# opencb/hpg-variant

Hardware: AMD Instinct MI355X
Metric: variants/s chi2 assoc (higher is better)
Workload: dtype u8

## Files before the change

hpg-variant_amd/csrc/hpgv_kernels.h:

```cpp
#pragma once
#include <hip/hip_runtime.h>
#include <stdint.h>

namespace hpgv {

__device__ __forceinline__ uint32_t nib_nonzero(uint32_t x) {
    uint32_t y = x | (x << 1);
    y = y | (y << 2);
    return y & 0x88888888u;
}
__device__ __forceinline__ uint32_t nib_not_f(uint32_t x) { return nib_nonzero(~x); }

__device__ __forceinline__ int wave_sum(int v) {
    v += __builtin_amdgcn_update_dpp(0, v, 0xB1, 0xF, 0xF, true);
    v += __builtin_amdgcn_update_dpp(0, v, 0x4E, 0xF, 0xF, true);
    v += __builtin_amdgcn_update_dpp(0, v, 0x141, 0xF, 0xF, true);
    v += __builtin_amdgcn_update_dpp(0, v, 0x140, 0xF, 0xF, true);
    return __builtin_amdgcn_readlane(v, 0) + __builtin_amdgcn_readlane(v, 16) +
           __builtin_amdgcn_readlane(v, 32) + __builtin_amdgcn_readlane(v, 48);
}

template <bool NT>
__device__ __forceinline__ uint4 load16(const uint4 *p);
template <bool NT>
__device__ __forceinline__ uint4 load16o(const uint8_t *__restrict__ base, uint32_t byte_off) {
    return load16<NT>(reinterpret_cast<const uint4 *>(base + byte_off));
}
template <bool NT>
__device__ __forceinline__ uint4 load16(const uint4 *p) {
    if constexpr (NT) {
        typedef uint32_t u32x4 __attribute__((ext_vector_type(4)));
        u32x4 t = __builtin_nontemporal_load(reinterpret_cast<const u32x4 *>(p));
        return make_uint4(t.x, t.y, t.z, t.w);
    } else {
        return *p;
    }
}

template <bool NT, int U, bool X>
__device__ __forceinline__ void assoc_row(const uint8_t *__restrict__ row, int lane, int chunksA,
                                          int chunks, uint32_t &pnz, uint32_t &pnnf, uint32_t &pbnz) {
    for (int base = 0; base < chunks; base += 64 * U) {
        uint4 q[U];
#pragma unroll
        for (int u = 0; u < U; ++u) {
            const int c = base + u * 64 + lane;
            q[u] = make_uint4(~0u, ~0u, ~0u, ~0u);
            if (c < chunks) q[u] = load16o<NT>(row, (uint32_t)c * 16u);
        }
#pragma unroll
        for (int u = 0; u < U; ++u) {
            const int c = base + u * 64 + lane;
            const uint32_t sh = (c < chunksA) ? 0u : 16u;
            const uint32_t w[4] = {q[u].x, q[u].y, q[u].z, q[u].w};
            uint32_t nz = 0, nnf = 0, bnz = 0;
#pragma unroll
            for (int k = 0; k < 4; ++k) {
                const uint32_t ind = nib_nonzero(w[k]);
                nz += __builtin_popcount(ind);
                nnf += __builtin_popcount(nib_not_f(w[k]));
                if constexpr (X) bnz += __builtin_popcount(ind & (ind >> 4) & 0x08080808u);
            }
            pnz += nz << sh;
            pnnf += nnf << sh;
            if constexpr (X) pbnz += bnz << sh;
        }
    }
}

__device__ __forceinline__ void assoc_row_finish(bool x_row, int lane, int TA, int TU, uint32_t pnz,
                                                 uint32_t pnnf, uint32_t pbnz, int4 *__restrict__ dst) {
    const int nzA = wave_sum((int)(pnz & 0xFFFFu)), nzU = wave_sum((int)(pnz >> 16));
    const int nfA = wave_sum((int)(pnnf & 0xFFFFu)), nfU = wave_sum((int)(pnnf >> 16));
    int4 out;
    if (!x_row) {
        out.x = TA - nzA;
        out.y = nzA + nfA - TA;
        out.z = TU - nzU;
        out.w = nzU + nfU - TU;
    } else {
        const int bA = wave_sum((int)(pbnz & 0xFFFFu)), bU = wave_sum((int)(pbnz >> 16));
        const int validA = nfA >> 1, validU = nfU >> 1;
        const int xxA = bA - (TA / 2 - validA), xxU = bU - (TU / 2 - validU);
        out.x = (TA - nzA) - validA + xxA;
        out.y = xxA;
        out.z = (TU - nzU) - validU + xxU;
        out.w = xxU;
    }
    if (lane == 0) *dst = out;
}

template <bool NT, int U, bool STRIDED>
__global__ __launch_bounds__(256) void k_assoc_scan(const uint8_t *__restrict__ gt, size_t pitch,
                                                    int n_variants, int chunksA, int chunks,
                                                    const uint8_t *__restrict__ is_x,
                                                    int4 *__restrict__ counts, int vpw) {
    const int lane = threadIdx.x & 63;
    const long wave = (long)blockIdx.x * (blockDim.x >> 6) + (threadIdx.x >> 6);
    const int slots = ((chunks + 64 * U - 1) / (64 * U)) * (64 * U);
    const int TA = 32 * chunksA;
    const int TU = 32 * (slots - chunksA);
    long v, v_end, v_step;
    if constexpr (STRIDED) { v = wave; v_end = n_variants; v_step = (long)gridDim.x * (blockDim.x >> 6); }
    else { v = wave * vpw; v_end = v + vpw < n_variants ? v + vpw : n_variants; v_step = 1; }

    for (; v < v_end; v += v_step) {
        const uint8_t *row = gt + (size_t)v * pitch;
        const bool x_row = (is_x != nullptr) && (__builtin_amdgcn_readfirstlane((int)is_x[v]) != 0);
        uint32_t pnz = 0, pnnf = 0, pbnz = 0;
        if (x_row) assoc_row<NT, U, true>(row, lane, chunksA, chunks, pnz, pnnf, pbnz);
        else       assoc_row<NT, U, false>(row, lane, chunksA, chunks, pnz, pnnf, pbnz);
        assoc_row_finish(x_row, lane, TA, TU, pnz, pnnf, pbnz, counts + v);
    }
}

struct AssocAcc { uint32_t pnz, pnnf, pbnz; };

template <int U, bool X>
__device__ __forceinline__ AssocAcc assoc_count_tile(const uint4 (&q)[U], int base, int lane, int chunksA,
                                                     AssocAcc a) {
#pragma unroll
    for (int u = 0; u < U; ++u) {
        const int c = base + u * 64 + lane;
        const uint32_t sh = (c < chunksA) ? 0u : 16u;
        const uint32_t w[4] = {q[u].x, q[u].y, q[u].z, q[u].w};
        uint32_t nz = 0, nnf = 0, bnz = 0;
#pragma unroll
        for (int k = 0; k < 4; ++k) {
            const uint32_t ind = nib_nonzero(w[k]);
            nz += __builtin_popcount(ind);
            nnf += __builtin_popcount(nib_not_f(w[k]));
            if constexpr (X) bnz += __builtin_popcount(ind & (ind >> 4) & 0x08080808u);
        }
        a.pnz += nz << sh;
        a.pnnf += nnf << sh;
        if constexpr (X) a.pbnz += bnz << sh;
    }
    return a;
}

template <bool NT, int U>
__device__ __forceinline__ void assoc_issue_tile(uint4 (&q)[U], const uint8_t *__restrict__ g0, size_t pitch,
                                                 int t, int ipr, int chunks, int lane) {
    const int r = t / ipr, base = (t - r * ipr) * 64 * U;
    const uint8_t *row = g0 + (size_t)r * pitch;
#pragma unroll
    for (int u = 0; u < U; ++u) {
        const int c = base + u * 64 + lane;
        q[u] = make_uint4(~0u, ~0u, ~0u, ~0u);
        if (c < chunks) q[u] = load16o<NT>(row, (uint32_t)c * 16u);
    }
}

template <int U>
__device__ __forceinline__ AssocAcc assoc_consume_tile(const uint4 (&q)[U], AssocAcc a, int t, int ipr, long v_begin,
                                                       int lane, int chunksA, int TA, int TU,
                                                       const uint8_t *__restrict__ is_x, int4 *__restrict__ counts) {
    const int r = t / ipr, it = t - r * ipr;
    const long v = v_begin + r;
    const bool x_row = (is_x != nullptr) && (__builtin_amdgcn_readfirstlane((int)is_x[v]) != 0);
    if (x_row) a = assoc_count_tile<U, true>(q, it * 64 * U, lane, chunksA, a);
    else       a = assoc_count_tile<U, false>(q, it * 64 * U, lane, chunksA, a);
    if (it == ipr - 1) {
        assoc_row_finish(x_row, lane, TA, TU, a.pnz, a.pnnf, a.pbnz, counts + v);
        a.pnz = a.pnnf = a.pbnz = 0;
    }
    return a;
}

template <bool NT, int U, int WAVES>
__global__ __launch_bounds__(256, WAVES) void k_assoc_scan_pipe(const uint8_t *__restrict__ gt, size_t pitch,
                                                         int n_variants, int chunksA, int chunks,
                                                         const uint8_t *__restrict__ is_x,
                                                         int4 *__restrict__ counts, int vpw) {
    const int lane = threadIdx.x & 63;
    const long wave = (long)blockIdx.x * (blockDim.x >> 6) + (threadIdx.x >> 6);
    const long v_begin = wave * vpw;
    if (v_begin >= n_variants) return;
    const int rows = (int)((v_begin + vpw <= n_variants) ? vpw : (n_variants - v_begin));
    const int ipr = (chunks + 64 * U - 1) / (64 * U);
    const int slots = ipr * 64 * U;
    const int TA = 32 * chunksA, TU = 32 * (slots - chunksA);
    const int n_tiles = rows * ipr;
    const uint8_t *g0 = gt + (size_t)v_begin * pitch;
    AssocAcc acc = {0u, 0u, 0u};
    uint4 qa[U], qb[U];
    assoc_issue_tile<NT, U>(qa, g0, pitch, 0, ipr, chunks, lane);
    for (int t = 0; t < n_tiles; t += 2) {
        if (t + 1 < n_tiles) assoc_issue_tile<NT, U>(qb, g0, pitch, t + 1, ipr, chunks, lane);
        acc = assoc_consume_tile<U>(qa, acc, t, ipr, v_begin, lane, chunksA, TA, TU, is_x, counts);
        if (t + 1 < n_tiles) {
            if (t + 2 < n_tiles) assoc_issue_tile<NT, U>(qa, g0, pitch, t + 2, ipr, chunks, lane);
            acc = assoc_consume_tile<U>(qb, acc, t + 1, ipr, v_begin, lane, chunksA, TA, TU, is_x, counts);
        }
    }
}

__device__ __forceinline__ double chisq_p_value(double x) {
    if (x != x) return x;
    if (x <= 0.0) return 1.0;
    const double y = x / 2.0;
    double P;
    if (y > 0.5) P = 1.0 - erfc(sqrt(y));
    else         P = erf(sqrt(y));
    return 1.0 - P;
}

__device__ __forceinline__ double assoc_odds(int A1, int A2, int U1, int U2) {
    return (A2 == 0 || U1 == 0) ? __builtin_nan("") : ((double)A1 / A2) * ((double)U2 / U1);
}

__device__ __forceinline__ double assoc_chisq_value(int a, int c, int b, int d) {
    const double total = a + c + b + d;
    const double t_aff = a + c, t_un = b + d, t_1 = a + b, t_2 = c + d;
    const double e_a1 = (t_aff * t_1) / total;
    const double e_a2 = (t_aff * t_2) / total;
    const double e_u1 = (t_un * t_1) / total;
    const double e_u2 = (t_un * t_2) / total;
    return ((a - e_a1) * (a - e_a1)) / e_a1 + ((c - e_a2) * (c - e_a2)) / e_a2 +
           ((b - e_u1) * (b - e_u1)) / e_u1 + ((d - e_u2) * (d - e_u2)) / e_u2;
}

static __global__ __launch_bounds__(256) void k_assoc_chisq(const int4 *__restrict__ counts, int n,
                                                     double *__restrict__ odds,
                                                     double *__restrict__ chisq,
                                                     double *__restrict__ pval) {
    const int i = blockIdx.x * blockDim.x + threadIdx.x;
    if (i >= n) return;
    const int4 c4 = counts[i];
    const int a = c4.x, c = c4.y, b = c4.z, d = c4.w;
    const double x = assoc_chisq_value(a, c, b, d);
    odds[i] = assoc_odds(a, c, b, d);
    chisq[i] = x;
    pval[i] = chisq_p_value(x);
}

__device__ __forceinline__ double wave_sum_f64(double v) {
#pragma unroll
    for (int off = 32; off > 0; off >>= 1) v += __shfl_xor(v, off);
    return v;
}
__device__ __forceinline__ double wave_max_f64(double v) {
#pragma unroll
    for (int off = 32; off > 0; off >>= 1) { const double o = __shfl_xor(v, off); v = o > v ? o : v; }
    return v;
}

__device__ const double k_exp2_j64[64] = {
    0x1.0000000000000p+0, 0x1.02c9a3e778061p+0, 0x1.059b0d3158574p+0, 0x1.0874518759bc8p+0,
    0x1.0b5586cf9890fp+0, 0x1.0e3ec32d3d1a2p+0, 0x1.11301d0125b51p+0, 0x1.1429aaea92de0p+0,
    0x1.172b83c7d517bp+0, 0x1.1a35beb6fcb75p+0, 0x1.1d4873168b9aap+0, 0x1.2063b88628cd6p+0,
    0x1.2387a6e756238p+0, 0x1.26b4565e27cddp+0, 0x1.29e9df51fdee1p+0, 0x1.2d285a6e4030bp+0,
    0x1.306fe0a31b715p+0, 0x1.33c08b26416ffp+0, 0x1.371a7373aa9cbp+0, 0x1.3a7db34e59ff7p+0,
    0x1.3dea64c123422p+0, 0x1.4160a21f72e2ap+0, 0x1.44e086061892dp+0, 0x1.486a2b5c13cd0p+0,
    0x1.4bfdad5362a27p+0, 0x1.4f9b2769d2ca7p+0, 0x1.5342b569d4f82p+0, 0x1.56f4736b527dap+0,
    0x1.5ab07dd485429p+0, 0x1.5e76f15ad2148p+0, 0x1.6247eb03a5585p+0, 0x1.6623882552225p+0,
    0x1.6a09e667f3bcdp+0, 0x1.6dfb23c651a2fp+0, 0x1.71f75e8ec5f74p+0, 0x1.75feb564267c9p+0,
    0x1.7a11473eb0187p+0, 0x1.7e2f336cf4e62p+0, 0x1.82589994cce13p+0, 0x1.868d99b4492edp+0,
    0x1.8ace5422aa0dbp+0, 0x1.8f1ae99157736p+0, 0x1.93737b0cdc5e5p+0, 0x1.97d829fde4e50p+0,
    0x1.9c49182a3f090p+0, 0x1.a0c667b5de565p+0, 0x1.a5503b23e255dp+0, 0x1.a9e6b5579fdbfp+0,
    0x1.ae89f995ad3adp+0, 0x1.b33a2b84f15fbp+0, 0x1.b7f76f2fb5e47p+0, 0x1.bcc1e904bc1d2p+0,
    0x1.c199bdd85529cp+0, 0x1.c67f12e57d14bp+0, 0x1.cb720dcef9069p+0, 0x1.d072d4a07897cp+0,
    0x1.d5818dcfba487p+0, 0x1.da9e603db3285p+0, 0x1.dfc97337b9b5fp+0, 0x1.e502ee78b3ff6p+0,
    0x1.ea4afa2a490dap+0, 0x1.efa1bee615a27p+0, 0x1.f50765b6e4540p+0, 0x1.fa7c1819e90d8p+0,
};
__device__ __forceinline__ double fisher_exp(double e, const double *tab ) {
    const double kf = __builtin_rint(e * 0x1.71547652b82fep+6);
    double r = __builtin_fma(-kf, 0x1.62e42fe000000p-7, e);
    r = __builtin_fma(-kf, 0x1.f473de6af278fp-36, r);
    const int ki = (int)kf;
    const double tj = tab[ki & 63];
    double q = __builtin_fma(r, 1.0 / 120.0, 1.0 / 24.0);
    q = __builtin_fma(r, q, 1.0 / 6.0);
    q = __builtin_fma(r, q, 0.5);
    q = __builtin_fma(r * r, q, r);
    const double y = __builtin_fma(tj, q, tj);
    return e < -1100.0 ? 0.0 : __builtin_ldexp(y, ki >> 6);
}

struct FisherTab {
    const double *lf; const double *xt ; double konst; int r1, c1, d0;
    __device__ __forceinline__ double at(uint32_t byte_off) const { return *reinterpret_cast<const double *>(reinterpret_cast<const char *>(lf) + byte_off); }
    __device__ __forceinline__ double e(int x) const {
        const uint32_t x8 = (uint32_t)x << 3;
        return konst - at(x8) - at(((uint32_t)r1 << 3) - x8) - at(((uint32_t)c1 << 3) - x8) - at(((uint32_t)d0 << 3) + x8);
    }
    __device__ __forceinline__ double p(int x) const { return fisher_exp(e(x), xt); }
    __device__ __forceinline__ void e2(int x, double *e0, double *e1) const {
        const char *b = reinterpret_cast<const char *>(lf) - 16;
        double2 q0, q1, q2, q3;
        __builtin_memcpy(&q0, b + ((uint32_t)(x + 2) << 3), 16);
        __builtin_memcpy(&q1, b + ((uint32_t)(r1 - x + 1) << 3), 16);
        __builtin_memcpy(&q2, b + ((uint32_t)(c1 - x + 1) << 3), 16);
        __builtin_memcpy(&q3, b + ((uint32_t)(d0 + x + 2) << 3), 16);
        *e0 = konst - q0.x - q1.y - q2.y - q3.x;
        *e1 = konst - q0.y - q1.x - q2.x - q3.y;
    }
};

template <int W> __device__ __forceinline__ int sub_lane(int lane) { return lane & (W - 1); }
template <int W> __device__ __forceinline__ uint64_t sub_ballot(bool pred, int lane) {
    const uint64_t b = __ballot(pred);
    if constexpr (W == 64) { (void)lane; return b; }
    else return (b >> (lane & ~(W - 1))) & ((1ull << W) - 1ull);
}
template <int W> __device__ __forceinline__ double sub_sum_f64(double v) {
#pragma unroll
    for (int off = W / 2; off > 0; off >>= 1) v += __shfl_xor(v, off);
    return v;
}
template <int W> __device__ __forceinline__ double sub_first_f64(double v, int lane) { return __shfl(v, lane & ~(W - 1)); }

template <int W>
__device__ __forceinline__ void fisher_boundaries(const FisherTab &T, double thr , int L1, int R1, int L2, int R2, int lane,
                                                  int *xL, int *xR) {
    const int sl = sub_lane<W>(lane);
    while (R1 - L1 > W || R2 - L2 > W) {
        const bool go1 = R1 - L1 > W, go2 = R2 - L2 > W;
        const int step1 = (R1 - L1 + W - 1) / W, step2 = (R2 - L2 + W - 1) / W;
        const int x1 = L1 + sl * step1, x2 = L2 + sl * step2;
        const double v1 = (go1 && x1 < R1) ? T.e(x1) : 0.0;
        const double v2 = (go2 && x2 < R2) ? T.e(x2) : 0.0;
        if (go1) {
            const int j = __builtin_popcountll(sub_ballot<W>(x1 < R1 && v1 <= thr, lane));
            const int xj = L1 + j * step1;
            const int nL = (j == 0) ? L1 : L1 + (j - 1) * step1 + 1, nR = (j == W || xj >= R1) ? R1 : xj;
            L1 = nL; R1 = nR;
        }
        if (go2) {
            const int j = __builtin_popcountll(sub_ballot<W>(x2 < R2 && v2 > thr, lane));
            const int xj = L2 + j * step2;
            const int nL = (j == 0) ? L2 : L2 + (j - 1) * step2 + 1, nR = (j == W || xj >= R2) ? R2 : xj;
            L2 = nL; R2 = nR;
        }
    }
    const int x1 = L1 + sl, x2 = L2 + sl;
    const double v1 = x1 < R1 ? T.e(x1) : 0.0, v2 = x2 < R2 ? T.e(x2) : 0.0;
    *xL = L1 + __builtin_popcountll(sub_ballot<W>(x1 < R1 && v1 <= thr, lane));
    *xR = L2 + __builtin_popcountll(sub_ballot<W>(x2 < R2 && v2 > thr, lane));
}

template <int W>
__device__ __forceinline__ double fisher_tails(const FisherTab &T, int xL, int xR, int lo, int hi, int lane, double rel_cut) {
    const int sl = sub_lane<W>(lane);
    double partL = 0.0, partR = 0.0, cutL = 0.0, cutR = 0.0;
    bool onL = true, onR = true;
    for (int k = 0; onL || onR; ++k) {
        const int firstL = xL - 1 - 2 * W * k, firstR = xR + 2 * W * k;
        if (firstL < lo) onL = false;
        if (firstR > hi) onR = false;
        const int a = firstL - 2 * sl, b = firstR + 2 * sl;
        double eL0 = -2000.0, eL1 = -2000.0, eR0 = -2000.0, eR1 = -2000.0;
        if (onL && a >= lo) { double lo_e, hi_e; T.e2(a - 1, &lo_e, &hi_e); eL0 = hi_e; if (a - 1 >= lo) eL1 = lo_e; }
        if (onR && b <= hi) { double lo_e, hi_e; T.e2(b, &lo_e, &hi_e); eR0 = lo_e; if (b + 1 <= hi) eR1 = hi_e; }
        const double sL0 = fisher_exp(eL0, T.xt), sL1 = fisher_exp(eL1, T.xt), sR0 = fisher_exp(eR0, T.xt), sR1 = fisher_exp(eR1, T.xt);
        partL += sL0 + sL1; partR += sR0 + sR1;
        if (k == 0) { cutL = rel_cut * sub_first_f64<W>(sL0, lane); cutR = rel_cut * sub_first_f64<W>(sR0, lane); }
        if (onL && sub_ballot<W>(sL0 > cutL || sL1 > cutL, lane) == 0ull) onL = false;
        if (onR && sub_ballot<W>(sR0 > cutR || sR1 > cutR, lane) == 0ull) onR = false;
    }
    return sub_sum_f64<W>(partL + partR);
}

template <int W>
__device__ __forceinline__ bool fisher_boundary_windows(const FisherTab &T, double thr , int mode, int obs, int lane,
                                                        int *L1, int *R1, int *L2, int *R2) {
    const int sl = sub_lane<W>(lane);
    const int g1 = obs <= mode ? obs + 1 : 2 * mode - obs + 1, g2 = obs <= mode ? 2 * mode - obs : obs;
    int w1 = g1 - W / 2, w2 = g2 - W / 2;
    w1 = w1 > *R1 - W ? *R1 - W : w1; w1 = w1 < *L1 ? *L1 : w1;
    w2 = w2 > *R2 - W ? *R2 - W : w2; w2 = w2 < *L2 ? *L2 : w2;
    const int x1 = w1 + sl, x2 = w2 + sl;
    const bool in1 = x1 < *R1, in2 = x2 < *R2;
    const double v1 = in1 ? T.e(x1) : 0.0, v2 = in2 ? T.e(x2) : 0.0;
    const int n1 = __builtin_popcountll(sub_ballot<W>(in1, lane)), n2 = __builtin_popcountll(sub_ballot<W>(in2, lane));
    const int c1 = __builtin_popcountll(sub_ballot<W>(in1 && v1 <= thr, lane)), c2 = __builtin_popcountll(sub_ballot<W>(in2 && v2 > thr, lane));
    bool ok = true;
    if (c1 == 0 && w1 > *L1) { *R1 = w1; ok = false; }
    else if (c1 == n1 && w1 + n1 < *R1) { *L1 = w1 + n1; ok = false; }
    else { *L1 = w1 + c1; *R1 = w1 + c1; }
    if (c2 == 0 && w2 > *L2) { *R2 = w2; ok = false; }
    else if (c2 == n2 && w2 + n2 < *R2) { *L2 = w2 + n2; ok = false; }
    else { *L2 = w2 + c2; *R2 = w2 + c2; }
    return ok;
}

template <int W>
__device__ __forceinline__ double fisher_sub(int a, int b, int c, int d, const double *__restrict__ lf,
                                             const double *exp_tab , double rel_cut, int lane) {
    const int sl = sub_lane<W>(lane);
    const int r1 = a + b, r2 = c + d, c1 = a + c, nn = r1 + r2;
    const int lo = (c1 - r2) > 0 ? (c1 - r2) : 0;
    const int hi = r1 < c1 ? r1 : c1;
    FisherTab T;
    T.lf = lf; T.xt = exp_tab; T.r1 = r1; T.c1 = c1; T.d0 = r2 - c1;
    T.konst = lf[r1] + lf[r2] + lf[c1] + lf[nn - c1] - lf[nn];
    const double thr = T.e(a) + 9.9999995000000333e-08;
    double sum;
    if (hi - lo < 8 * W) {
        double part = 0.0;
        for (int x = lo + sl; x <= hi; x += W) {
            const double ex = T.e(x);
            if (ex <= thr) part += fisher_exp(ex, exp_tab);
        }
        sum = sub_sum_f64<W>(part);
    } else {
        const double prod = (double)(r1 + 1) * (double)(c1 + 1), den = (double)(nn + 2);
        double md = __builtin_floor(prod / den);
        const double rem = __builtin_fma(-md, den, prod);
        md += rem >= den ? 1.0 : (rem < 0.0 ? -1.0 : 0.0);
        int mode = (int)md;
        mode = mode < lo ? lo : (mode > hi ? hi : mode);
        int L1 = lo, R1 = mode + 1, L2 = mode + 1, R2 = hi + 1, xL, xR;
        if (fisher_boundary_windows<W>(T, thr, mode, a, lane, &L1, &R1, &L2, &R2)) { xL = L1; xR = L2; }
        else fisher_boundaries<W>(T, thr, L1, R1, L2, R2, lane, &xL, &xR);
        sum = fisher_tails<W>(T, xL, xR, lo, hi, lane, rel_cut);
    }
    return sum > 1.0 ? 1.0 : sum;
}

__device__ __forceinline__ double fisher_wave(int a, int b, int c, int d, const double *__restrict__ lf,
                                              const double *exp_tab , double rel_cut, int lane) {
    return fisher_sub<64>(a, b, c, d, lf, exp_tab, rel_cut, lane);
}

template <int W>
__global__ __launch_bounds__(256) void k_assoc_fisher(const int4 *__restrict__ counts, int n,
                                                      const double *__restrict__ lf,
                                                      double *__restrict__ odds,
                                                      double *__restrict__ pval, double rel_cut) {
    __shared__ double exp_tab[64];
    if (threadIdx.x < 64) exp_tab[threadIdx.x] = k_exp2_j64[threadIdx.x];
    __syncthreads();
    const int lane = threadIdx.x & 63;
    constexpr int PER_WAVE = 64 / W;
    const long wave = (long)blockIdx.x * (blockDim.x >> 6) + (threadIdx.x >> 6);
    const long v = wave * PER_WAVE + lane / W;
    if (v >= n) return;
    const int4 c4 = counts[v];
    const int a = c4.x, b = c4.y, c = c4.z, d = c4.w;
    const double p = fisher_sub<W>(a, b, c, d, lf, exp_tab, rel_cut, lane);
    if (sub_lane<W>(lane) == 0) {
        odds[v] = assoc_odds(a, b, c, d);
        pval[v] = p;
    }
}

__host__ __device__ __forceinline__ uint64_t splitmix64(uint64_t x) {
    x ^= x >> 30; x *= 0xbf58476d1ce4e5b9ULL;
    x ^= x >> 27; x *= 0x94d049bb133111ebULL;
    x ^= x >> 31;
    return x;
}
#define HPGV_SYNTH_SEED 0x4850475631ULL

static __global__ void k_synth_thresholds(uint64_t v0, int n, uint32_t *__restrict__ thr) {
    const int i = blockIdx.x * blockDim.x + threadIdx.x;
    if (i >= n) return;
    const uint64_t v = v0 + (uint64_t)i;
    const uint64_t h = splitmix64(HPGV_SYNTH_SEED ^ 0xA11E1EULL ^ v);
    const double u = (double)(h >> 11) * (1.0 / 9007199254740992.0);
    const double q = 0.05 + 0.45 * u;
    const uint32_t t_miss = 167772u;
    const double rest = (double)(16777216u - t_miss);
    const double omq = 1.0 - q;
    const double p00 = omq * omq;
    const double p01 = 2.0 * q * omq;
    const uint32_t t00 = t_miss + (uint32_t)floor(p00 * rest);
    const uint32_t t01 = t00 + (uint32_t)floor(p01 * rest);
    thr[3 * i + 0] = t_miss; thr[3 * i + 1] = t00; thr[3 * i + 2] = t01;
}

__device__ __forceinline__ uint32_t synth_gt(uint64_t vterm, uint64_t s, uint32_t tm, uint32_t t0,
                                             uint32_t t1) {
    const uint32_t r = (uint32_t)(splitmix64(vterm + s) >> 40);
    return (r < tm) ? 0xFFu : (r < t0) ? 0x00u : (r < t1) ? 0x01u : 0x11u;
}

enum { RECODE_NONE = 0, RECODE_TDT = 1, RECODE_STATS = 2, RECODE_MENDEL = 3, RECODE_EPI = 4 };

constexpr uint32_t TDT_F_UNUSABLE = 0x80u, TDT_M_UNUSABLE = 0x20u;
constexpr uint32_t TDT_C_INVALID = 4u;

__host__ __device__ __forceinline__ uint32_t tdt_parent_class(uint32_t g, uint32_t unusable) {
    const uint32_t a1 = g >> 4, a2 = g & 0xFu;
    if (a1 == 0xFu || a2 == 0xFu) return unusable;
    if (a1 && !a2) return unusable;
    if (!a1 && !a2) return 0u;
    if (!a1) return 1u;
    return (a1 == a2) ? 2u : 3u;
}
__host__ __device__ __forceinline__ uint32_t tdt_child_class(uint32_t g) {
    const uint32_t a1 = g >> 4, a2 = g & 0xFu;
    if (a1 == 0xFu || a2 == 0xFu) return TDT_C_INVALID;
    if (!a1 && !a2) return 0u;
    if (!a1) return 1u;
    if (!a2) return 2u;
    return 3u;
}
__host__ __device__ __forceinline__ uint32_t stats_flags(uint32_t g) {
    const uint32_t a1 = g >> 4, a2 = g & 0xFu;
    uint32_t f = 0;
    if (g == 0x00u) f |= 1u; else if (g == 0x01u) f |= 2u; else if (g == 0x10u) f |= 4u; else if (g == 0x11u) f |= 8u;
    if (a1 == 0xFu || a2 == 0xFu) f |= 0x10u;
    if (a1 == 0xFu && a2 == 0xFu) f |= 0x20u;
    if (!(f & 0xFu)) {
        if (a1 == 0u || a2 == 0u) f |= 0x40u;
        if (a1 == 1u || a2 == 1u) f |= 0x80u;
    }
    return f;
}

__host__ __device__ __forceinline__ uint32_t mendel_class(uint32_t g) {
    const uint32_t a1 = g >> 4, a2 = g & 0xFu;
    if (a1 == 0xFu || a2 == 0xFu) return 3u;
    if (!a1 && !a2) return 0u;
    return (a1 && a2) ? 2u : 1u;
}

__device__ __forceinline__ uint32_t recode_byte(uint32_t g, int mode, int p16, int pos, bool is_pad) {
    if (mode == RECODE_TDT) {
        if (p16 <= 0 || pos >= 3 * p16) return g;
        if (pos < p16) return tdt_parent_class(g, TDT_F_UNUSABLE);
        if (pos < 2 * p16) return tdt_parent_class(g, TDT_M_UNUSABLE);
        return tdt_child_class(g);
    }
    if (mode == RECODE_STATS) return is_pad ? 0u : stats_flags(g);
    if (mode == RECODE_MENDEL) return mendel_class(g);
    if (mode == RECODE_EPI) {
        const uint32_t a1 = g >> 4, a2 = g & 0xFu;
        if (a1 == 0xFu || a2 == 0xFu) return 255u;
        if (!a1 && !a2) return 0u;
        if (a1 != a2) return 1u;
        return 2u;
    }
    return g;
}

static __global__ __launch_bounds__(256) void k_synth_layout(uint64_t v0, int n_variants, size_t pitch,
                                                      int chunks, const int32_t *__restrict__ col_of_pos,
                                                      const uint32_t *__restrict__ thr, int mode, int p16,
                                                      uint8_t *__restrict__ dst) {
    const long t = (long)blockIdx.x * blockDim.x + threadIdx.x;
    const long total = (long)n_variants * chunks;
    if (t >= total) return;
    const int i = (int)(t / chunks), c = (int)(t % chunks);
    const uint64_t v = v0 + (uint64_t)i;
    const uint64_t vterm = HPGV_SYNTH_SEED + v * 0x9E3779B97F4A7C15ULL;
    const uint32_t tm = thr[3 * i], t0 = thr[3 * i + 1], t1 = thr[3 * i + 2];
    uint32_t w[4];
#pragma unroll
    for (int k = 0; k < 4; ++k) {
        uint32_t acc = 0;
#pragma unroll
        for (int j = 0; j < 4; ++j) {
            const int pos = c * 16 + k * 4 + j;
            const int col = col_of_pos[pos];
            uint32_t g = (col < 0) ? 0xFFu : synth_gt(vterm, (uint64_t)col, tm, t0, t1);
            g = recode_byte(g, mode, p16, pos, col < 0);
            acc |= g << (8 * j);
        }
        w[k] = acc;
    }
    *reinterpret_cast<uint4 *>(dst + (size_t)i * pitch + (size_t)c * 16) = make_uint4(w[0], w[1], w[2], w[3]);
}

static __global__ __launch_bounds__(256) void k_layout(const uint8_t *__restrict__ src, size_t src_pitch,
                                                int n_variants, size_t pitch, int chunks,
                                                const int32_t *__restrict__ col_of_pos, int strict,
                                                int mode, int p16, uint8_t *__restrict__ dst) {
    const long t = (long)blockIdx.x * blockDim.x + threadIdx.x;
    const long total = (long)n_variants * chunks;
    if (t >= total) return;
    const int i = (int)(t / chunks), c = (int)(t % chunks);
    const uint8_t *row = src + (size_t)i * src_pitch;
    uint32_t w[4];
#pragma unroll
    for (int k = 0; k < 4; ++k) {
        uint32_t acc = 0;
#pragma unroll
        for (int j = 0; j < 4; ++j) {
            const int pos = c * 16 + k * 4 + j;
            const int col = col_of_pos[pos];
            uint32_t g = (col < 0) ? 0xFFu : (uint32_t)row[col];
            if (strict && (((g & 0xF) == 0xF) || ((g >> 4) == 0xF))) g = 0xFFu;
            g = recode_byte(g, mode, p16, pos, col < 0);
            acc |= g << (8 * j);
        }
        w[k] = acc;
    }
    *reinterpret_cast<uint4 *>(dst + (size_t)i * pitch + (size_t)c * 16) = make_uint4(w[0], w[1], w[2], w[3]);
}

static __global__ void k_counts_to_soa(const int4 *__restrict__ counts, int n, int32_t *A1, int32_t *A2,
                                int32_t *U1, int32_t *U2) {
    const int i = blockIdx.x * blockDim.x + threadIdx.x;
    if (i >= n) return;
    const int4 c = counts[i];
    A1[i] = c.x; A2[i] = c.y; U1[i] = c.z; U2[i] = c.w;
}

template <bool NT>
__global__ __launch_bounds__(256) void k_read_probe(const uint4 *__restrict__ buf, size_t n16,
                                                    uint32_t *__restrict__ sink) {
    const int lane = threadIdx.x & 63;
    const size_t wave = (size_t)blockIdx.x * (blockDim.x >> 6) + (threadIdx.x >> 6);
    const size_t n_waves = (size_t)gridDim.x * (blockDim.x >> 6);
    const size_t piece = 512;
    uint32_t acc = 0;
    uint4 qa[8], qb[8];
    size_t p = wave * piece;
    auto issue = [&](uint4 (&q)[8], size_t base) {
#pragma unroll
        for (int u = 0; u < 8; ++u) {
            const size_t i = base + (size_t)u * 64 + lane;
            q[u] = make_uint4(0, 0, 0, 0);
            if (i < n16) q[u] = load16<NT>(buf + i);
        }
    };
    auto eat = [&](const uint4 (&q)[8]) {
#pragma unroll
        for (int u = 0; u < 8; ++u) acc |= q[u].x | q[u].y | q[u].z | q[u].w;
    };
    if (p < n16) issue(qa, p);
    while (p < n16) {
        const size_t p1 = p + n_waves * piece;
        if (p1 < n16) issue(qb, p1);
        eat(qa);
        if (p1 >= n16) break;
        const size_t p2 = p1 + n_waves * piece;
        if (p2 < n16) issue(qa, p2);
        eat(qb);
        p = p2;
    }
    if (acc == 0x12345678u) sink[0] = acc;
}

}
```

Before: 136.5 million.

## Restructure Fisher tail summation with strength-reduced offsets and last-lane termination

Rewrites the Fisher exact test tail loop to precompute per-lane byte offsets into the log-factorial table and step them with a wave-uniform stride, replacing per-iteration index arithmetic and bounds checks with precomputed iteration limits. Early termination now looks only at the outermost term of each sub-wave (the last lane's second sample) through a ballot/inverse-ballot broadcast, instead of checking every lane's terms. The underflow clamp in the exp helper is removed to shorten the inner path. The main risk is out-of-range lanes: they now load table entries and rely on limit checks, and very negative exponents now depend on ldexp underflow behaviour.

```diff
diff --git a/hpg-variant_amd/csrc/hpgv_kernels.h b/hpg-variant_amd/csrc/hpgv_kernels.h
--- a/hpg-variant_amd/csrc/hpgv_kernels.h
+++ b/hpg-variant_amd/csrc/hpgv_kernels.h
@@ -275,7 +275,7 @@
     q = __builtin_fma(r, q, 0.5);
     q = __builtin_fma(r * r, q, r);
     const double y = __builtin_fma(tj, q, tj);
-    return e < -1100.0 ? 0.0 : __builtin_ldexp(y, ki >> 6);
+    return __builtin_ldexp(y, ki >> 6);
 }
 
 struct FisherTab {
@@ -286,6 +286,12 @@
         return konst - at(x8) - at(((uint32_t)r1 << 3) - x8) - at(((uint32_t)c1 << 3) - x8) - at(((uint32_t)d0 << 3) + x8);
     }
     __device__ __forceinline__ double p(int x) const { return fisher_exp(e(x), xt); }
+    static __device__ __forceinline__ double2 at2(const char *base, uint32_t &byte_off) {
+        asm volatile("" : "+v"(byte_off));
+        double2 q;
+        __builtin_memcpy(&q, base + byte_off, 16);
+        return q;
+    }
     __device__ __forceinline__ void e2(int x, double *e0, double *e1) const {
         const char *b = reinterpret_cast<const char *>(lf) - 16;
         double2 q0, q1, q2, q3;
@@ -310,6 +316,13 @@
     return v;
 }
 template <int W> __device__ __forceinline__ double sub_first_f64(double v, int lane) { return __shfl(v, lane & ~(W - 1)); }
+template <int W> __device__ __forceinline__ bool sub_last_pred(bool pred) {
+    constexpr uint64_t LAST = (W == 64 ? 1ull : W == 32 ? 0x0000000100000001ull : W == 16 ? 0x0001000100010001ull : 0x0101010101010101ull) << (W - 1);
+    uint64_t m = __builtin_amdgcn_ballot_w64(pred) & LAST;
+#pragma unroll
+    for (int s = 1; s < W; s <<= 1) m |= m >> s;
+    return __builtin_amdgcn_inverse_ballot_w64(m);
+}
 
 template <int W>
 __device__ __forceinline__ void fisher_boundaries(const FisherTab &T, double thr , int L1, int R1, int L2, int R2, int lane,
@@ -342,22 +355,42 @@
 
 template <int W>
 __device__ __forceinline__ double fisher_tails(const FisherTab &T, int xL, int xR, int lo, int hi, int lane, double rel_cut) {
+    constexpr int SH = W == 64 ? 7 : (W == 32 ? 6 : (W == 16 ? 5 : 4));
+    static_assert((1 << SH) == 2 * W, "sub-wave widths: 8, 16, 32, 64");
+    constexpr long STEP = 2L * W * 8;
     const int sl = sub_lane<W>(lane);
+    const int a0 = xL - 1 - 2 * sl, b0 = xR + 2 * sl;
+    const int limL0 = (a0 - lo) >> SH, limL1 = (a0 - 1 - lo) >> SH, limR0 = (hi - b0) >> SH, limR1 = (hi - b0 - 1) >> SH;
+    uint32_t oL0 = (uint32_t)(a0 + 1) << 3, oL1 = (uint32_t)(T.r1 - a0 + 2) << 3, oL2 = (uint32_t)(T.c1 - a0 + 2) << 3, oL3 = (uint32_t)(T.d0 + a0 + 1) << 3;
+    uint32_t oR0 = (uint32_t)(b0 + 2) << 3, oR1 = (uint32_t)(T.r1 - b0 + 1) << 3, oR2 = (uint32_t)(T.c1 - b0 + 1) << 3, oR3 = (uint32_t)(T.d0 + b0 + 2) << 3;
+    const char *base = reinterpret_cast<const char *>(T.lf) - 16;
     double partL = 0.0, partR = 0.0, cutL = 0.0, cutR = 0.0;
     bool onL = true, onR = true;
-    for (int k = 0; onL || onR; ++k) {
-        const int firstL = xL - 1 - 2 * W * k, firstR = xR + 2 * W * k;
-        if (firstL < lo) onL = false;
-        if (firstR > hi) onR = false;
-        const int a = firstL - 2 * sl, b = firstR + 2 * sl;
-        double eL0 = -2000.0, eL1 = -2000.0, eR0 = -2000.0, eR1 = -2000.0;
-        if (onL && a >= lo) { double lo_e, hi_e; T.e2(a - 1, &lo_e, &hi_e); eL0 = hi_e; if (a - 1 >= lo) eL1 = lo_e; }
-        if (onR && b <= hi) { double lo_e, hi_e; T.e2(b, &lo_e, &hi_e); eR0 = lo_e; if (b + 1 <= hi) eR1 = hi_e; }
-        const double sL0 = fisher_exp(eL0, T.xt), sL1 = fisher_exp(eL1, T.xt), sR0 = fisher_exp(eR0, T.xt), sR1 = fisher_exp(eR1, T.xt);
-        partL += sL0 + sL1; partR += sR0 + sR1;
-        if (k == 0) { cutL = rel_cut * sub_first_f64<W>(sL0, lane); cutR = rel_cut * sub_first_f64<W>(sR0, lane); }
-        if (onL && sub_ballot<W>(sL0 > cutL || sL1 > cutL, lane) == 0ull) onL = false;
-        if (onR && sub_ballot<W>(sR0 > cutR || sR1 > cutR, lane) == 0ull) onR = false;
+    for (int k = 0;; ++k) {
+        const long kb = (long)__builtin_amdgcn_readfirstlane(k) * STEP;
+        const char *dn = base - kb, *up = base + kb;
+        const bool liveL = onL && k <= limL0, liveR = onR && k <= limR0;
+        if (!(liveL || liveR)) break;
+        if (liveL) {
+            const double2 q0 = FisherTab::at2(dn, oL0), q1 = FisherTab::at2(up, oL1), q2 = FisherTab::at2(up, oL2), q3 = FisherTab::at2(dn, oL3);
+            const double e0 = T.konst - q0.y - q1.x - q2.x - q3.y;
+            const double e1 = T.konst - q0.x - q1.y - q2.y - q3.x;
+            const double s0 = fisher_exp(e0, T.xt);
+            const double t1 = fisher_exp(e1, T.xt), s1 = k <= limL1 ? t1 : 0.0;
+            partL += s0 + s1;
+            if (k == 0) cutL = rel_cut * sub_first_f64<W>(s0, lane);
+            onL = sub_last_pred<W>(s1 > cutL);
+        }
+        if (liveR) {
+            const double2 q0 = FisherTab::at2(up, oR0), q1 = FisherTab::at2(dn, oR1), q2 = FisherTab::at2(dn, oR2), q3 = FisherTab::at2(up, oR3);
+            const double e0 = T.konst - q0.x - q1.y - q2.y - q3.x;
+            const double e1 = T.konst - q0.y - q1.x - q2.x - q3.y;
+            const double s0 = fisher_exp(e0, T.xt);
+            const double t1 = fisher_exp(e1, T.xt), s1 = k <= limR1 ? t1 : 0.0;
+            partR += s0 + s1;
+            if (k == 0) cutR = rel_cut * sub_first_f64<W>(s0, lane);
+            onR = sub_last_pred<W>(s1 > cutR);
+        }
     }
     return sub_sum_f64<W>(partL + partR);
 }
```

New measurement: 137.0 million, median of 4. No clear change (+0.4%).
